# Eclectic-Sheep/sheeprl

Hardware: NVIDIA H100
Metric: Dreamer-V3 train-steps/sec (S, bs16 seq64 horizon15, 64x64x3 obs) (higher is better)
Workload: dtype f32

## Files before the change

sheeprl_b200/csrc/rssm_scan.cu:

```cuda
#include "b200rl.h"
#include "common.cuh"

namespace {

constexpr int SCAN_G = 128;
constexpr int SCAN_NT = 512;
constexpr int SCAN_NW = SCAN_NT / 32;
constexpr int MAXB = 16;
constexpr int MAXRPU = 8;
constexpr int KS_MAX = 8;
constexpr int CLS_SLICES = 8;

typedef unsigned long long u64;

__host__ __device__ inline int r4(int x) { return (x + 3) / 4 * 4; }
__host__ __device__ inline int imax(int a, int b) { return a > b ? a : b; }
__host__ __device__ inline int imin(int a, int b) { return a < b ? a : b; }

__host__ __device__ inline int owned_groups(int width, int cta) {
  const int groups = (width + 3) / 4;
  return (groups > cta) ? (groups - cta + SCAN_G - 1) / SCAN_G : 0;
}
__host__ __device__ inline int owned_cols(int width, int cta) {
  int n = 0;
// ... 147 lines not shown
                make_float2(__uint_as_float((unsigned)a[u]), __uint_as_float((unsigned)b[u]));
      }
    }
  if (!has_s) return;
  while (poll_sums() && !sp.fail()) {}
  float v0 = 0.f, v1 = 0.f;
#pragma unroll
  for (int i = 0; i < SCAN_G / 32; ++i) {
    v0 += __uint_as_float((unsigned)sx[i]);
    v1 += __uint_as_float((unsigned)sy[i]);
  }
  v0 = warp_sum(v0); v1 = warp_sum(v1);
  if (lane == 0) { out1[sr0 + wid] = v0 * inv; out2[sr0 + wid] = v1 * inv; }
}

struct Slot {
  int b, cj, col;
  bool ok;
};
__device__ __forceinline__ Slot make_slot(int e, int per_row, int B, int cta, int width) {
  Slot s;
  s.b = per_row > 0 ? e / per_row : 0;
  s.cj = e - s.b * per_row;
  s.col = (cta + (s.cj >> 2) * SCAN_G) * 4 + (s.cj & 3);
  s.ok = per_row > 0 && s.b < B && s.col < width;
  return s;
}

__device__ __forceinline__ float fsilu(float x) { return __fdividef(x, 1.f + __expf(-x)); }

__device__ __forceinline__ void mma_tf32(float (&d)[4], const unsigned (&a)[4], unsigned b0, unsigned b1) {
  asm volatile("mma.sync.aligned.m16n8k8.row.col.f32.tf32.tf32.f32 {%0,%1,%2,%3}, {%4,%5,%6,%7}, {%8,%9}, {%0,%1,%2,%3};"
               : "+f"(d[0]), "+f"(d[1]), "+f"(d[2]), "+f"(d[3])
               : "r"(a[0]), "r"(a[1]), "r"(a[2]), "r"(a[3]), "r"(b0), "r"(b1));
}
__device__ __forceinline__ unsigned tf32_hi(float x) { return __float_as_uint(x) & 0xffffe000u; }
__device__ __forceinline__ unsigned tf32_lo(float x) { return __float_as_uint(x - __uint_as_float(__float_as_uint(x) & 0xffffe000u)); }

__device__ __forceinline__ void mma_item(const float* __restrict__ X, int xs, int B, const float* __restrict__ w, int wst,
                                         int nvalid, int k0, int k1, float* part, int ldp, int c0, int lane) {
  const int g = lane >> 2, t = lane & 3;
  const bool r_lo = g < B, r_hi = g + 8 < B, n_ok = g < nvalid;
  const float* xa = X + (size_t)g * xs;
  const float* xb = X + (size_t)(g + 8) * xs;
  const float* wr = w + (size_t)g * wst;
  float d[4] = {0.f, 0.f, 0.f, 0.f}, dx[4] = {0.f, 0.f, 0.f, 0.f}, dy[4] = {0.f, 0.f, 0.f, 0.f};
  for (int kb = k0; kb < k1; kb += 16) {
    const int k = kb + 4 * t;
    const bool k_ok = k < k1;
    float4 va = make_float4(0.f, 0.f, 0.f, 0.f), vb = va, vw = va;
    if (r_lo && k_ok) va = *reinterpret_cast<const float4*>(xa + k);
    if (r_hi && k_ok) vb = *reinterpret_cast<const float4*>(xb + k);
    if (n_ok && k_ok) vw = *reinterpret_cast<const float4*>(wr + k);
    {
      const unsigned ah[4] = {tf32_hi(va.x), tf32_hi(vb.x), tf32_hi(va.y), tf32_hi(vb.y)};
      const unsigned al[4] = {tf32_lo(va.x), tf32_lo(vb.x), tf32_lo(va.y), tf32_lo(vb.y)};
      const unsigned bh0 = tf32_hi(vw.x), bh1 = tf32_hi(vw.y), bl0 = tf32_lo(vw.x), bl1 = tf32_lo(vw.y);
      mma_tf32(dx, ah, bl0, bl1);
      mma_tf32(dy, al, bh0, bh1);
      mma_tf32(d, ah, bh0, bh1);
    }
    {
      const unsigned ah[4] = {tf32_hi(va.z), tf32_hi(vb.z), tf32_hi(va.w), tf32_hi(vb.w)};
      const unsigned al[4] = {tf32_lo(va.z), tf32_lo(vb.z), tf32_lo(va.w), tf32_lo(vb.w)};
      const unsigned bh0 = tf32_hi(vw.z), bh1 = tf32_hi(vw.w), bl0 = tf32_lo(vw.z), bl1 = tf32_lo(vw.w);
      mma_tf32(dx, ah, bl0, bl1);
      mma_tf32(dy, al, bh0, bh1);
      mma_tf32(d, ah, bh0, bh1);
    }
  }
#pragma unroll
  for (int i = 0; i < 4; ++i) d[i] += dx[i] + dy[i];
  const int c = 2 * t;
  if (c < nvalid) {
    part[(size_t)g * ldp + c0 + c] = d[0];
    part[(size_t)(g + 8) * ldp + c0 + c] = d[2];
  }
  if (c + 1 < nvalid) {
    part[(size_t)g * ldp + c0 + c + 1] = d[1];
    part[(size_t)(g + 8) * ldp + c0 + c + 1] = d[3];
  }
}

__device__ __forceinline__ int product(const float* X, int xs, const float* wbase, int wst, int ngroups, int K, int B,
                                       float* PART, int ldp, int cbase, int tid) {
  if (ngroups <= 0) return 0;
  const int lane = tid & 31, wid = tid >> 5;
  const int ncols = ngroups * 4, ntiles = (ncols + 7) >> 3, Kp = r4(K);
  int ks = imin(KS_MAX, imax(1, SCAN_NW / ntiles));
  const int kchunk = ((Kp + ks - 1) / ks + 15) / 16 * 16;
  ks = (Kp + kchunk - 1) / kchunk;
  for (int item = wid; item < ntiles * ks; item += SCAN_NW) {
    const int sl = item / ntiles, tile = item - sl * ntiles;
    const int k0 = sl * kchunk, k1 = imin(Kp, k0 + kchunk);
    mma_item(X, xs, B, wbase + (size_t)tile * 8 * wst, wst, imin(8, ncols - tile * 8), k0, k1,
             PART + (size_t)sl * MAXB * ldp, ldp, cbase + tile * 8, lane);
  }
  return ks;
}

__device__ __forceinline__ float part_sum(const float* PART, int ldp, int ks, int b, int c) {
  float v = 0.f;
  for (int s = 0; s < ks; ++s) v += PART[((size_t)s * MAXB + b) * ldp + c];
  return v;
}

__device__ __forceinline__ void class_product(const float* X, int xs, const float* W, int wst, int D, int Kp, int nr, float* PART,
                                              int tid) {
  const int lane = tid & 31, wid = tid >> 5, g = lane >> 2, t = lane & 3;
  const int sl = wid % CLS_SLICES, half = wid / CLS_SLICES;
  const int kc = ((Kp + CLS_SLICES - 1) / CLS_SLICES + 15) / 16 * 16;
  const int k0 = sl * kc, k1 = imin(Kp, k0 + kc);
  const int n0 = half * 16;
  if (n0 >= D) return;
  const bool r_ok = g < nr, n_ok0 = n0 + g < D, n_ok1 = n0 + 8 + g < D;
  const float* xa = X + (size_t)g * xs;
  const float* w0 = W + (size_t)(n0 + g) * wst;
  const float* w1 = W + (size_t)(n0 + 8 + g) * wst;
  float d0[4] = {0.f, 0.f, 0.f, 0.f}, d1[4] = {0.f, 0.f, 0.f, 0.f};
  float e0[4] = {0.f, 0.f, 0.f, 0.f}, e1[4] = {0.f, 0.f, 0.f, 0.f};
  for (int kb = k0; kb < k1; kb += 16) {
    const int k = kb + 4 * t;
    const bool k_ok = k < k1;
    float4 va = make_float4(0.f, 0.f, 0.f, 0.f), v0 = va, v1 = va;
    if (r_ok && k_ok) va = *reinterpret_cast<const float4*>(xa + k);
    if (n_ok0 && k_ok) v0 = *reinterpret_cast<const float4*>(w0 + k);
    if (n_ok1 && k_ok) v1 = *reinterpret_cast<const float4*>(w1 + k);
    {
      const unsigned ah[4] = {tf32_hi(va.x), 0u, tf32_hi(va.y), 0u}, al[4] = {tf32_lo(va.x), 0u, tf32_lo(va.y), 0u};
      mma_tf32(e0, ah, tf32_lo(v0.x), tf32_lo(v0.y)); mma_tf32(e1, ah, tf32_lo(v1.x), tf32_lo(v1.y));
      mma_tf32(d0, ah, tf32_hi(v0.x), tf32_hi(v0.y)); mma_tf32(d1, ah, tf32_hi(v1.x), tf32_hi(v1.y));
      mma_tf32(e0, al, tf32_hi(v0.x), tf32_hi(v0.y)); mma_tf32(e1, al, tf32_hi(v1.x), tf32_hi(v1.y));
    }
    {
      const unsigned ah[4] = {tf32_hi(va.z), 0u, tf32_hi(va.w), 0u}, al[4] = {tf32_lo(va.z), 0u, tf32_lo(va.w), 0u};
      mma_tf32(e0, ah, tf32_lo(v0.z), tf32_lo(v0.w)); mma_tf32(e1, ah, tf32_lo(v1.z), tf32_lo(v1.w));
      mma_tf32(d0, ah, tf32_hi(v0.z), tf32_hi(v0.w)); mma_tf32(d1, ah, tf32_hi(v1.z), tf32_hi(v1.w));
      mma_tf32(e0, al, tf32_hi(v0.z), tf32_hi(v0.w)); mma_tf32(e1, al, tf32_hi(v1.z), tf32_hi(v1.w));
    }
  }
  if (g < nr) {
    float* out = PART + ((size_t)sl * MAXRPU + g) * 32 + n0 + 2 * t;
    out[0] = d0[0] + e0[0]; out[1] = d0[1] + e0[1];
    out[8] = d1[0] + e1[0]; out[9] = d1[1] + e1[1];
  }
}

__device__ __forceinline__ void load_rows4(float* dst, int wst, int koff, const float* W, size_t ld, int row0, int nrows_valid,
                                           int c0, int K, int Kp, int tid) {
  for (int j = 0; j < 4; ++j)
    for (int k = tid; k < Kp; k += SCAN_NT)
      dst[j * wst + koff + k] = (row0 + j < nrows_valid && k < K) ? W[(size_t)(row0 + j) * ld + c0 + k] : 0.f;
}
__device__ __forceinline__ void load_cols4(float* dst, int wst, const float* W, size_t ld, int col0, int ncols_valid,
                                           int K, int koff, int tid) {
  for (int e = tid; e < K * 4; e += SCAN_NT) {
    const int k = e >> 2, j = e & 3;
    dst[j * wst + koff + k] = (col0 + j < ncols_valid) ? W[(size_t)k * ld + col0 + j] : 0.f;
  }
}

__device__ __forceinline__ void prof_mark(long long* prof, int slot, long long& last, bool on) {
  if (on) {
    const long long now = clock64();
    prof[slot] += now - last;
    last = now;
  }
}

struct GeoF {
  int ngh, ngr, ngx;
  int sR, sDx, sDr, wgst, w2st;
  int nsplit, rpu;
  int unit_g, unit_r0, unit_nr;
  int ldp;
  int kin;
  int oWg, oWr1, oW2, oWin, oXh, oXx, oPart, oAcc, oX0, oPar, oMisc, oInt, total;
};

struct Dims { int B, S, D, R, Dx, Dr, A; };

// ... 333 lines not shown
      prof_mark(prof, 10, tlast, prof_on);
      {
        const int nrp = nr <= 1 ? 1 : (nr <= 2 ? 2 : (nr <= 4 ? 4 : 8));
        const int wpr = SCAN_NW / nrp, bb = wid / wpr, wi = wid - bb * wpr;
        float* xr = Xx + bb * xxs;
        float s = 0.f, q2 = 0.f;
        if (bb < nr)
          for (int k = wi * 32 + lane; k < Dr; k += wpr * 32) { const float xv = xr[k]; s += xv; q2 = fmaf(xv, xv, q2); }
        s = warp_sum(s);
        q2 = warp_sum(q2);
        if (lane == 0) { misc[48 + wid] = s; misc[80 + wid] = q2; }
        __syncthreads();
        float mu = 0.f, var = 0.f;
        for (int i = 0; i < wpr; ++i) { mu += misc[48 + bb * wpr + i]; var += misc[80 + bb * wpr + i]; }
        mu /= (float)Dr;
        var = fmaxf(var / (float)Dr - mu * mu, 0.f);
        const float rstd = rsqrtf(var + a.eps);
        if (bb < nr) {
          for (int k = wi * 32 + lane; k < Dr; k += wpr * 32) {
            const float o = fsilu((xr[k] - mu) * rstd * LNRG[k] + LNRB[k]);
            xr[k] = o;
            if (gq == 0) a.rp_act[(row0 + rb + bb) * Dr + k] = o;
          }
          if (gq == 0 && wi == 0 && lane == 0) {
            ws.ln_stats[((size_t)2 * NB + row0 + rb + bb) * 2] = mu;
            ws.ln_stats[((size_t)2 * NB + row0 + rb + bb) * 2 + 1] = rstd;
          }
        }
      }
      __syncthreads();
      prof_mark(prof, 14, tlast, prof_on);
      class_product(Xx, xxs, W2, g.w2st, D, g.sDr, nr, PART, tid);
      __syncthreads();
      prof_mark(prof, 15, tlast, prof_on);
      if (wid < nr) {
        const int bb = wid, b = rb + bb;
        const bool on = lane < D;
        float lg = 0.f;
        for (int s2 = 0; s2 < CLS_SLICES; ++s2) lg += PART[((size_t)s2 * MAXRPU + bb) * 32 + lane];
        const float raw = on ? lg + bias2 : -INFINITY;
        const float mx = warp_max(raw);
        const float ex = on ? expf(raw - mx) : 0.f;
        const float se = warp_sum(ex);
        float pmc = ex / se, l = raw;
        if (a.unimix > 0.f) {
          pmc = fminf(fmaxf((1.f - a.unimix) * pmc + a.unimix / (float)D, kFp32Eps), 1.f - kFp32Eps);
          l = logf(pmc);
        }
        float best = on ? pmc / noise_pref : -INFINITY;
        int besti = on ? lane : 0x7fffffff;
#pragma unroll
        for (int s2 = 16; s2 > 0; s2 >>= 1) {
          const float ob = __shfl_xor_sync(0xffffffffu, best, s2);
          const int oi = __shfl_xor_sync(0xffffffffu, besti, s2);
          if (ob > best || (ob == best && oi < besti)) { best = ob; besti = oi; }
        }
        if (lane == 0) ll_store(ws.ll + L.z + ((size_t)par * MAXB + b) * S + gq, __uint_as_float((unsigned)besti), tag);
        const size_t o = (row0 + b) * Z + (size_t)gq * D + lane;
        if (lane == 0) ws.zidx[(row0 + b) * S + gq] = besti;
        if (on) {
          a.post_raw[o] = raw;
          a.post_mix[o] = l;
          const float zt = (lane == besti) ? 1.f : 0.f;
          a.latent[(row0 + b) * a.ld_lat + (size_t)gq * D + lane] = zt;
          if (t + 1 < T)
            a.z_in[(row0 + B + b) * Z + (size_t)gq * D + lane] = (1.f - fnext) * zt + fnext * ((z0idx[gq] == lane) ? 1.f : 0.f);
        }
      }
      prof_mark(prof, 11, tlast, prof_on);
    }
    __syncthreads();
    if (sp.dead) break;
  }
  if (prof_on)
    for (int i = 0; i < 32; ++i) ws.prof[cta * 32 + i] = sprof[i];
}

struct GeoB {
  int ngh, ngx, ngr;
  int sZ, sR, sDx, sDr, xw;
  int wgst, winst;
  int nsplit, rpu, unit_g, unit_r0, unit_nr;
  int ldp;
  int oW2, oW1, oWg, oWin, oX, oPart, oAcc, oSt, oDhc, oDh0, oWs, oMisc, total;
};

__host__ __device__ inline GeoB make_geo_b(const Dims& a, int cta) {
  GeoB g;
  const int Z = a.S * a.D;
  g.ngh = owned_groups(a.R, cta);
  g.ngx = owned_groups(a.Dx, cta);
  g.ngr = owned_groups(a.Dr, cta);
  g.sZ = r4(Z); g.sR = r4(a.R); g.sDx = r4(a.Dx); g.sDr = r4(a.Dr);
  g.xw = imax(imax(g.sZ, 2 * g.sR), imax(g.sDx, g.sDr));
  g.wgst = 3 * g.sR;
  g.winst = g.sDx + 4;
  g.nsplit = imax(1, imin(a.B, SCAN_G / a.S));
  g.rpu = (a.B + g.nsplit - 1) / g.nsplit;
  g.unit_g = -1; g.unit_r0 = 0; g.unit_nr = 0;
  if (cta < a.S * g.nsplit) {
    const int sp = cta / a.S;
    g.unit_r0 = sp * g.rpu;
    g.unit_nr = imin(g.rpu, a.B - g.unit_r0);
    if (g.unit_nr > 0) g.unit_g = cta % a.S; else g.unit_nr = 0;
  }
  const int mh = owned_groups(a.R, 0), mx = owned_groups(a.Dx, 0), mr = owned_groups(a.Dr, 0);
  g.ldp = imax(imax((mh + mx) * 4, mr * 4), 4);
  int o = 0;
  g.oW2 = o;   o += mr * 4 * g.sZ;
  g.oW1 = o;   o += mh * 4 * g.sDr;
  g.oWg = o;   o += (mh + mx) * 4 * g.wgst;
  g.oWin = o;  o += a.D * g.winst;
  g.oX = o;    o += MAXB * g.xw;
  g.oPart = o; o += imax(KS_MAX * MAXB * g.ldp, CLS_SLICES * MAXRPU * 32);
  g.oAcc = o;  o += MAXB * g.ldp;
  g.oSt = o;   o += 2 * MAXB * imax(imax(mh * 12, mx * 4), imax(mr * 4, 4));
  g.oDhc = o;  o += MAXB * imax(mh * 4, 4);
  g.oDh0 = o;  o += imax(mh * 4, 4);
  g.oWs = o;   o += mh * 4 + (mh + mx) * 4 + 32;
  g.oMisc = o; o += 16 * MAXB + 64;
  g.total = o;
  return g;
}

__device__ __forceinline__ void send_row_sums(const float* ST, int ncols, int B, u64* base, int par, int cta, unsigned tag, int tid) {
  const int lane = tid & 31, wid = tid >> 5;
  for (int b = wid; b < B; b += SCAN_NW) {
    float s1 = 0.f, s2 = 0.f;
    for (int c = lane; c < ncols; c += 32) { s1 += ST[(b * ncols + c) * 2]; s2 += ST[(b * ncols + c) * 2 + 1]; }
    s1 = warp_sum(s1); s2 = warp_sum(s2);
    if (lane == 0) ll_store2(base + (((size_t)par * MAXB + b) * SCAN_G + cta) * 2, s1, s2, tag);
  }
}

template <bool FIX>
__global__ void __launch_bounds__(SCAN_NT, 1)
rssm_scan_bwd_kernel(const b200rl_rssm_scan_args a, const b200rl_rssm_scan_grads q) {
  extern __shared__ __align__(16) float sm[];
  const int tid = threadIdx.x, lane = tid & 31, wid = tid >> 5;
  const int cta = blockIdx.x;
  const int T = a.T, B = a.B;
  const int S = FIX ? 32 : a.S, D = FIX ? 32 : a.D, Z = S * D, R = FIX ? 512 : a.R, Dx = FIX ? 512 : a.Dx, Dr = FIX ? 512 : a.Dr;
  const int KG = R + Dx, KIN = Z + a.A, NB = T * B;
  const GeoB g = make_geo_b(Dims{B, S, D, R, Dx, Dr, a.A}, cta);
  const Workspace ws = carve(a.workspace, T, B, S, D, Dx, R, Dr);
  const LLGeo L = make_ll(S, Dx, R, Dr, Z);
  const int mh = owned_groups(R, 0), mx = owned_groups(Dx, 0);
  float* W2T = sm + g.oW2;
  float* W1T = sm + g.oW1;
  float* WgT = sm + g.oWg;
  float* WinU = sm + g.oWin;
  float* X = sm + g.oX;
  float* PART = sm + g.oPart;
  float* ACC = sm + g.oAcc;
  float* ST = sm + g.oSt;
  float* DHC = sm + g.oDhc;
  float* DH0 = sm + g.oDh0;
  float* WS1 = sm + g.oWs;
  float* WSG = WS1 + mh * 4;
  float* WSI = WSG + (mh + mx) * 4;
  float* misc = sm + g.oMisc;
  float* S1 = misc + 32;
  float* S2 = misc + 48;
  float* LNS = misc + 64;
  float* LNX1 = misc + 64 + 6 * MAXB;
  const int xw = g.xw, ldp = g.ldp;
  const int nh4 = g.ngh * 4, nx4 = g.ngx * 4, nr4 = g.ngr * 4;
  const bool unit = g.unit_g >= 0;
  __shared__ long long sprof[32];
  const bool prof_on = (cta < 2) && tid == 0;
  long long* prof = sprof;
  if (tid < 32) sprof[tid] = 0;
  long long tlast = prof_on ? clock64() : 0;
  Spin sp;
  sp.init(ws.error);

  for (int e = tid; e < g.total; e += SCAN_NT) sm[e] = 0.f;
  __syncthreads();
  for (int gi = 0; gi < g.ngr; ++gi)
    load_cols4(W2T + (size_t)gi * 4 * g.sZ, g.sZ, a.W_r2, Dr, (cta + gi * SCAN_G) * 4, Dr, Z, 0, tid);
  for (int gi = 0; gi < g.ngh; ++gi) {
    const int c0 = (cta + gi * SCAN_G) * 4;
    load_cols4(W1T + (size_t)gi * 4 * g.sDr, g.sDr, a.W_r1, a.ld_wr1, c0, R, Dr, 0, tid);
    for (int part = 0; part < 3; ++part)
      load_cols4(WgT + (size_t)gi * 4 * g.wgst, g.wgst, a.W_g + (size_t)part * R * KG, KG, c0, R, R, part * g.sR, tid);
  }
  for (int gi = 0; gi < g.ngx; ++gi)
    for (int part = 0; part < 3; ++part)
      load_cols4(WgT + (size_t)(g.ngh + gi) * 4 * g.wgst, g.wgst, a.W_g + (size_t)part * R * KG + R, KG,
                 (cta + gi * SCAN_G) * 4, Dx, R, part * g.sR, tid);
  if (unit)
    for (int e = tid; e < D * Dx; e += SCAN_NT) {
      const int c = e / D, d = e - c * D;
      WinU[d * g.winst + c] = a.W_in[(size_t)c * KIN + g.unit_g * D + d];
    }
  __syncthreads();
  for (int j = wid; j < nh4; j += SCAN_NW) {
    float s = 0.f;
    for (int k = lane; k < g.sDr; k += 32) s += W1T[(size_t)j * g.sDr + k];
    s = warp_sum(s);
    if (lane == 0) WS1[j] = s;
  }
  for (int j = wid; j < nh4 + nx4; j += SCAN_NW) {
    float s = 0.f;
    for (int k = lane; k < g.wgst; k += 32) s += WgT[(size_t)j * g.wgst + k];
    s = warp_sum(s);
    if (lane == 0) WSG[j] = s;
  }
  if (unit)
    for (int d = wid; d < D; d += SCAN_NW) {
      float s = 0.f;
      for (int k = lane; k < g.sDx; k += 32) s += WinU[(size_t)d * g.winst + k];
      s = warp_sum(s);
      if (lane == 0) WSI[d] = s;
    }
  __syncthreads();
  const Slot sR_ = make_slot(tid, nr4, B, cta, Dr);
  const Slot sH = make_slot(tid, nh4, B, cta, R);
  const Slot sX = make_slot(tid, nx4, B, cta, Dx);
  const float gam_r = sR_.ok ? a.lnr_g[sR_.col] : 0.f, bet_r = sR_.ok ? a.lnr_b[sR_.col] : 0.f;
  const float gam_x = sX.ok ? a.lnx_g[sX.col] : 0.f, bet_x = sX.ok ? a.lnx_b[sX.col] : 0.f;
  float gam_g[3] = {0.f, 0.f, 0.f};
  if (sH.ok)
#pragma unroll
    for (int part = 0; part < 3; ++part) gam_g[part] = a.lng_g[part * R + sH.col];
  const float ws1 = sH.ok ? WS1[sH.cj] : 0.f, wsgh = sH.ok ? WSG[sH.cj] : 0.f, wsgx = sX.ok ? WSG[nh4 + sX.cj] : 0.f;
  const float wsi = (unit && lane < D) ? WSI[lane] : 0.f;
  float dh0_acc = 0.f;
  prof_mark(prof, 16, tlast, prof_on);

  for (int t = T - 1; t >= 0; --t) {
    const size_t row0 = (size_t)t * B;
    const int bt = T - 1 - t, par = bt & 1;
    const unsigned tag = (unsigned)bt + 1u;
    const bool last = (t == T - 1);

    if (tid < MAXB) {
      misc[tid] = (tid < B) ? a.first[row0 + tid] : 0.f;
      misc[16 + tid] = (tid < B && !last) ? a.first[row0 + B + tid] : 0.f;
    }
    for (int e = tid; e < 3 * B * 2; e += SCAN_NT) {
      const int which = e / (B * 2), r_ = e - which * (B * 2);
      LNS[which * MAXB * 2 + r_] = ws.ln_stats[((size_t)which * NB + row0) * 2 + r_];
    }
    if (!last)
      for (int e = tid; e < B * 2; e += SCAN_NT) LNX1[e] = ws.ln_stats[((size_t)0 * NB + row0 + B) * 2 + e];
    const float p_rp = sR_.ok ? a.rp_pre[(row0 + sR_.b) * Dr + sR_.col] : 0.f;
    float p_hin = 0.f, p_dlh = 0.f, p_qr = 0.f, p_qgh = 0.f, p_gl[3] = {0.f, 0.f, 0.f}, p_gp[3] = {0.f, 0.f, 0.f};
    if (sH.ok) {
      p_hin = a.h_in[(row0 + sH.b) * R + sH.col];
      p_dlh = q.d_latent[(row0 + sH.b) * a.ld_lat + Z + sH.col];
      p_qr = q.q_r[(row0 + sH.b) * R + sH.col];
      p_qgh = q.q_g[(row0 + sH.b) * KG + sH.col];
#pragma unroll
      for (int part = 0; part < 3; ++part) {
        p_gl[part] = a.g_ln[(row0 + sH.b) * 3 * R + part * R + sH.col];
        p_gp[part] = a.g_pre[(row0 + sH.b) * 3 * R + part * R + sH.col];
      }
    }
    const float p_xp = sX.ok ? a.x_pre[(row0 + sX.b) * Dx + sX.col] : 0.f;
    const float p_qgx = sX.ok ? q.q_g[(row0 + sX.b) * KG + R + sX.col] : 0.f;
    float u_dl = 0.f, u_dmix = 0.f, u_raw = -INFINITY, u_qx = 0.f;
    if (unit && wid < g.unit_nr && lane < D) {
      const size_t o = (row0 + g.unit_r0 + wid) * Z + (size_t)g.unit_g * D + lane;
      u_dl = q.d_latent[(row0 + g.unit_r0 + wid) * a.ld_lat + (size_t)g.unit_g * D + lane];
      u_dmix = q.d_post_mix[o];
      u_raw = a.post_raw[o];
      if (!last) u_qx = q.q_x[(row0 + B + g.unit_r0 + wid) * Z + (size_t)g.unit_g * D + lane];
    }
    __syncthreads();
    const float* fl = misc;

    if (unit) {
      const int gq = g.unit_g, nr = g.unit_nr, rb = g.unit_r0;
      if (!last) {
        ll_recv<4>(X, xw, ws.ll + L.d + ((size_t)(par ^ 1) * MAXB + rb) * Dx, Dx, nr, Dx, (unsigned)bt, tid, sp,
                   ws.ll + L.sd + (size_t)(par ^ 1) * MAXB * SCAN_G * 2, rb, 1.f / (float)Dx, S1, S2);
        __syncthreads();
        prof_mark(prof, 17, tlast, prof_on);
        class_product(X, xw, WinU, g.winst, D, g.sDx, nr, PART, tid);
        __syncthreads();
      }
      if (wid < nr) {
        const int bb = wid, b = rb + bb;
        const bool on = lane < D;
        float dz = u_dl;
        if (!last) {
          float p1 = 0.f;
          for (int s2 = 0; s2 < CLS_SLICES; ++s2) p1 += PART[((size_t)s2 * MAXRPU + bb) * 32 + lane];
          if (on) {
            const float mu = LNX1[b * 2], rstd = LNX1[b * 2 + 1];
            const float p2 = rstd * (u_qx - mu * wsi);
            dz += (1.f - fl[16 + b]) * rstd * (p1 - S1[b] * wsi - S2[b] * p2);
          }
        }
        const float mx_ = warp_max(u_raw);
        const float ex = on ? expf(u_raw - mx_) : 0.f;
        const float sft = ex / warp_sum(ex);
        float gg = u_dmix;
        if (a.unimix > 0.f) {
          const float pmx = (1.f - a.unimix) * sft + a.unimix / (float)D;
          const float pmc = on ? fminf(fmaxf(pmx, kFp32Eps), 1.f - kFp32Eps) : 0.f;
          const float p = pmc / warp_sum(pmc);
          const float pdz = warp_sum(p * dz);
          gg += p * (dz - pdz);
          const bool inside = on && pmx >= kFp32Eps && pmx <= 1.f - kFp32Eps;
          const float ds = inside ? gg * (1.f - a.unimix) / pmx : 0.f;
          const float sds = warp_sum(sft * ds);
          gg = sft * (ds - sds);
        } else {
          const float pdz = warp_sum(sft * dz);
          gg += sft * (dz - pdz);
        }
        if (on) {
          ll_store(ws.ll + L.a + ((size_t)par * MAXB + b) * Z + (size_t)gq * D + lane, gg, tag);
          q.d_post_raw[(row0 + b) * Z + (size_t)gq * D + lane] = gg;
        }
      }
      prof_mark(prof, 18, tlast, prof_on);
    }

    __syncthreads();
    ll_recv<4>(X, xw, ws.ll + L.a + (size_t)par * MAXB * Z, Z, B, Z, tag, tid, sp);
    __syncthreads();
    prof_mark(prof, 19, tlast, prof_on);
    const int ks2 = product(X, xw, W2T, g.sZ, g.ngr, Z, B, PART, ldp, 0, tid);
    __syncthreads();
    float dact_r = 0.f;
    if (sR_.ok) {
      dact_r = part_sum(PART, ldp, ks2, sR_.b, sR_.cj);
      const float xh = (p_rp - LNS[(2 * MAXB + sR_.b) * 2]) * LNS[(2 * MAXB + sR_.b) * 2 + 1];
      const float ln = xh * gam_r + bet_r;
      const float sg = sigmoidf_(ln);
      const float dxh = dact_r * sg * (1.f + ln * (1.f - sg)) * gam_r;
      ll_store(ws.ll + L.b + ((size_t)par * MAXB + sR_.b) * Dr + sR_.col, dxh, tag);
      ST[(sR_.b * nr4 + sR_.cj) * 2] = dxh;
      ST[(sR_.b * nr4 + sR_.cj) * 2 + 1] = dxh * xh;
    } else if (tid < B * nr4) {
      ST[tid * 2] = 0.f; ST[tid * 2 + 1] = 0.f;
    }
    __syncthreads();
    send_row_sums(ST, nr4, B, ws.ll + L.sb, par, cta, tag, tid);
    if (sR_.ok) q.d_rp_act[(row0 + sR_.b) * Dr + sR_.col] = dact_r;
    prof_mark(prof, 20, tlast, prof_on);

    __syncthreads();
    ll_recv<4>(X, xw, ws.ll + L.b + (size_t)par * MAXB * Dr, Dr, B, Dr, tag, tid, sp,
               ws.ll + L.sb + (size_t)par * MAXB * SCAN_G * 2, 0, 1.f / (float)Dr, S1, S2);
    __syncthreads();
    prof_mark(prof, 21, tlast, prof_on);
    const int ks1 = product(X, xw, W1T, g.sDr, g.ngh, Dr, B, PART, ldp, 0, tid);
    __syncthreads();
    float dhin_gate = 0.f, dgl[3] = {0.f, 0.f, 0.f};
    if (sH.ok) {
      const int b = sH.b;
      const float mur = LNS[(2 * MAXB + b) * 2], rstdr = LNS[(2 * MAXB + b) * 2 + 1];
      const float mug = LNS[(1 * MAXB + b) * 2], rstdg = LNS[(1 * MAXB + b) * 2 + 1];
      const float p1 = part_sum(PART, ldp, ks1, b, sH.cj);
      const float p2 = rstdr * (p_qr - mur * ws1);
      float dh = p_dlh + rstdr * (p1 - S1[b] * ws1 - S2[b] * p2);
      if (!last) dh += DHC[b * nh4 + sH.cj];
      const float r = sigmoidf_(p_gl[0]), cnd = tanhf(r * p_gl[1]), u = sigmoidf_(p_gl[2] - 1.f);
      const float du = dh * (cnd - p_hin);
      const float drc = dh * u * (1.f - cnd * cnd);
      dgl[0] = drc * p_gl[1] * r * (1.f - r);
      dgl[1] = drc * r;
      dgl[2] = du * u * (1.f - u);
      dhin_gate = dh * (1.f - u);
#pragma unroll
      for (int part = 0; part < 3; ++part) {
        const float xh = (p_gp[part] - mug) * rstdg;
        const float dxh = dgl[part] * gam_g[part];
        ll_store(ws.ll + L.c + ((size_t)par * MAXB + b) * 3 * R + (size_t)part * R + sH.col, dxh, tag);
        ST[(b * (3 * nh4) + part * nh4 + sH.cj) * 2] = dxh;
        ST[(b * (3 * nh4) + part * nh4 + sH.cj) * 2 + 1] = dxh * xh;
      }
    } else if (tid < B * nh4) {
      const int b = tid / imax(nh4, 1), cj = tid - b * nh4;
#pragma unroll
      for (int part = 0; part < 3; ++part) {
        ST[(b * (3 * nh4) + part * nh4 + cj) * 2] = 0.f;
        ST[(b * (3 * nh4) + part * nh4 + cj) * 2 + 1] = 0.f;
      }
    }
    __syncthreads();
    send_row_sums(ST, 3 * nh4, B, ws.ll + L.sc, par, cta, tag, tid);
    if (sH.ok)
#pragma unroll
      for (int part = 0; part < 3; ++part) q.d_g_ln[(row0 + sH.b) * 3 * R + part * R + sH.col] = dgl[part];
    prof_mark(prof, 22, tlast, prof_on);

    __syncthreads();
    for (int part = 0; part < 2; ++part)
      ll_recv<4>(X + part * g.sR, xw, ws.ll + L.c + (size_t)par * MAXB * 3 * R + (size_t)part * R, 3 * R, B, R, tag, tid, sp);
    __syncthreads();
    const int ksa = product(X, xw, WgT, g.wgst, g.ngh + g.ngx, 2 * g.sR, B, PART, ldp, 0, tid);
    __syncthreads();
    float acc_h = sH.ok ? part_sum(PART, ldp, ksa, sH.b, sH.cj) : 0.f;
    float acc_x = sX.ok ? part_sum(PART, ldp, ksa, sX.b, nh4 + sX.cj) : 0.f;
    __syncthreads();
    ll_recv<4>(X, xw, ws.ll + L.c + (size_t)par * MAXB * 3 * R + (size_t)2 * R, 3 * R, B, R, tag, tid, sp,
               ws.ll + L.sc + (size_t)par * MAXB * SCAN_G * 2, 0, 1.f / (float)(3 * R), S1, S2);
    __syncthreads();
    const int ksb = product(X, xw, WgT + 2 * g.sR, g.wgst, g.ngh + g.ngx, R, B, PART, ldp, 0, tid);
    __syncthreads();
    prof_mark(prof, 23, tlast, prof_on);
    float dact_x = 0.f;
    if (sX.ok) {
      const int b = sX.b;
      acc_x += part_sum(PART, ldp, ksb, b, nh4 + sX.cj);
      const float mug = LNS[(1 * MAXB + b) * 2], rstdg = LNS[(1 * MAXB + b) * 2 + 1];
      const float mux = LNS[(0 * MAXB + b) * 2], rstdx = LNS[(0 * MAXB + b) * 2 + 1];
      const float p2 = rstdg * (p_qgx - mug * wsgx);
      dact_x = rstdg * (acc_x - S1[b] * wsgx - S2[b] * p2);
      const float xh = (p_xp - mux) * rstdx;
      const float ln = xh * gam_x + bet_x;
      const float sg = sigmoidf_(ln);
      const float dxh = dact_x * sg * (1.f + ln * (1.f - sg)) * gam_x;
      ll_store(ws.ll + L.d + ((size_t)par * MAXB + b) * Dx + sX.col, dxh, tag);
      ST[(b * nx4 + sX.cj) * 2] = dxh;
      ST[(b * nx4 + sX.cj) * 2 + 1] = dxh * xh;
    } else if (tid < B * nx4) {
      ST[tid * 2] = 0.f; ST[tid * 2 + 1] = 0.f;
    }
    float dhin_f = 0.f;
    if (sH.ok) {
      const int b = sH.b;
      acc_h += part_sum(PART, ldp, ksb, b, sH.cj);
      const float mug = LNS[(1 * MAXB + b) * 2], rstdg = LNS[(1 * MAXB + b) * 2 + 1];
      const float p2 = rstdg * (p_qgh - mug * wsgh);
      const float dhin = dhin_gate + rstdg * (acc_h - S1[b] * wsgh - S2[b] * p2);
      DHC[b * nh4 + sH.cj] = (1.f - fl[b]) * dhin;
      dhin_f = fl[b] * dhin;
    }
    __syncthreads();
    send_row_sums(ST, nx4, B, ws.ll + L.sd, par, cta, tag, tid);
    if (sX.ok) q.d_x_act[(row0 + sX.b) * Dx + sX.col] = dact_x;
    if (sH.ok) ACC[sH.b * ldp + sH.cj] = dhin_f;
    __syncthreads();
    if (tid < nh4)
      for (int b = 0; b < B; ++b)
        if (fl[b] != 0.f) dh0_acc += ACC[b * ldp + tid];
    prof_mark(prof, 24, tlast, prof_on);
    __syncthreads();
    if (sp.dead) break;
  }
  if (tid < nh4) {
    const int col = (cta + (tid >> 2) * SCAN_G) * 4 + (tid & 3);
    if (col < R) q.d_h0[col] = dh0_acc;
  }
  (void)DH0;
  if (prof_on)
    for (int i = 0; i < 32; ++i) ws.prof[cta * 32 + i] = sprof[i];
}

bool fixed_dims(const b200rl_rssm_scan_args& a) { return a.S == 32 && a.D == 32 && a.R == 512 && a.Dx == 512 && a.Dr == 512; }

size_t scan_smem(const b200rl_rssm_scan_args& a, bool backward) {
  const Dims d{a.B, a.S, a.D, a.R, a.Dx, a.Dr, a.A};
  return sizeof(float) * (size_t)(backward ? make_geo_b(d, 0).total : make_geo_f(d, 0).total);
}

int scan_check(const b200rl_rssm_scan_args& a, bool backward) {
  RL_CHECK_ARG(a.B >= 1 && a.B <= MAXB, "persistent scan supports batch <= 16 rows per rank");
  RL_CHECK_ARG(a.D >= 1 && a.D <= 32, "persistent scan supports <= 32 classes per categorical");
  RL_CHECK_ARG(a.T >= 1 && a.S >= 1 && a.S <= 64, "persistent scan supports T >= 1 and 1 <= S <= 64 categoricals");
  RL_CHECK_ARG(a.Dx % 2 == 0 && a.R % 2 == 0 && a.Dr % 2 == 0 && (a.S * a.D) % 2 == 0, "persistent scan supports even layer widths");
  RL_CHECK_ARG(a.Dx <= 1024, "persistent scan supports recurrent dense_units <= 1024");
  RL_CHECK_ARG(MAXB * owned_groups(a.R, 0) * 12 <= SCAN_NT, "persistent scan supports recurrent_state_size <= 1024");
  RL_CHECK_ARG(MAXB * owned_groups(a.Dr, 0) * 4 <= SCAN_NT, "persistent scan supports representation hidden_size <= 4096");
  RL_CHECK_ARG(scan_smem(a, backward) <= 227 * 1024, "weight slices do not fit in shared memory for this model size");
  return B200RL_OK;
}

int workspace_check(const b200rl_rssm_scan_args& a) {
  RL_CHECK_ARG(a.workspace && a.workspace_bytes >= (long long)ws_bytes(a.T, a.B, a.S, a.D, a.Dx, a.R, a.Dr), "workspace too small");
  return B200RL_OK;
}

struct GruLL { size_t s, h, c, sc, total; };
__host__ __device__ inline GruLL make_gru_ll(int R) {
  GruLL g;
  size_t o = 0;
  g.s = o;  o += 2 * (size_t)MAXB * SCAN_G * 2;
  g.h = o;  o += 2 * (size_t)MAXB * R;
  g.c = o;  o += 2 * (size_t)MAXB * 3 * R;
  g.sc = o; o += 2 * (size_t)MAXB * SCAN_G * 2;
  g.total = o;
  return g;
}
__host__ __device__ inline size_t gru_ws_bytes(int T, int B, int R) {
  return WS_HEADER + make_gru_ll(R).total * sizeof(u64) + sizeof(float) * 2 * (size_t)T * B + 256;
}

struct GeoG {
  int ngh, sR, ldp;
  int pw;
  int oW, oX, oPart, oAcc, oSt, oDhc, oPar, oLn, oMisc, oTab, total;
};
__host__ __device__ inline GeoG make_geo_g(int R, int cta, bool backward) {
  GeoG g;
  g.ngh = owned_groups(R, cta);
  g.sR = r4(R);
  const int mh = owned_groups(R, 0);
  g.ldp = backward ? mh * 4 : mh * 12;
  for (g.pw = backward ? 3 : 1;; g.pw = 1) {
    int o = 0;
    g.oW = o;    o += mh * 12 * g.sR;
    g.oX = o;    o += MAXB * g.pw * g.sR;
    g.oPart = o; o += KS_MAX * MAXB * g.ldp;
    g.oAcc = o;  o += MAXB * g.ldp;
    g.oSt = o;   o += backward ? 2 * MAXB * mh * 12 : 0;
// ... 393 lines not shown
```

Before: 62.17.

## Fuse gate-gradient products and poll low-latency flags inside the MMA loop

The backward scan's two sequential gate-gradient products (first two gate parts, then the third part after a separate receive) become one fused work list. Warps consume the third part directly from the tagged low-latency buffer, polling the tags inside the MMA item, which removes a receive phase and two block barriers per timestep. LayerNorm gamma/beta and weight sums move from registers into shared memory to relieve register pressure. The PART buffer doubles in size, which raises shared memory use, and spin-polling inside warps could serialize on slow producers.

```diff
diff --git a/sheeprl_b200/csrc/rssm_scan.cu b/sheeprl_b200/csrc/rssm_scan.cu
--- a/sheeprl_b200/csrc/rssm_scan.cu
+++ b/sheeprl_b200/csrc/rssm_scan.cu
@@ -253,14 +253,104 @@
   }
 }
 
+template <int LL_STEPS>
+__device__ __forceinline__ void mma_item_ll(const u64* src, int ss, int kvalid, int B, const float* __restrict__ w, int wst,
+                                            int nvalid, int k0, int k1, float* part, int ldp, int c0, int lane, unsigned tag,
+                                            Spin& sp) {
+  const int g = lane >> 2, t = lane & 3;
+  const bool r_lo = g < B, r_hi = g + 8 < B, n_ok = g < nvalid;
+  const u64* xa = src + (size_t)g * ss;
+  const u64* xb = src + (size_t)(g + 8) * ss;
+  const float* wr = w + (size_t)g * wst;
+  float d[4] = {0.f, 0.f, 0.f, 0.f}, dx[4] = {0.f, 0.f, 0.f, 0.f}, dy[4] = {0.f, 0.f, 0.f, 0.f};
+  const u64 zero = ll_pack(0.f, tag);
+  for (int kb0 = k0; kb0 < k1; kb0 += 16 * LL_STEPS) {
+    u64 e[LL_STEPS][8];
+    auto polled = [&](int s, int p) {
+      const int k = kb0 + 16 * s + 4 * t + 2 * (p & 1);
+      return ((p >> 1) ? r_hi : r_lo) && k < k1 && k < kvalid;
+    };
+    auto load = [&](int s, int p) {
+      const int k = kb0 + 16 * s + 4 * t + 2 * (p & 1);
+      ll_load2(((p >> 1) ? xb : xa) + k, e[s][2 * p], e[s][2 * p + 1]);
+    };
+#pragma unroll
+    for (int s = 0; s < LL_STEPS; ++s)
+#pragma unroll
+      for (int p = 0; p < 4; ++p) {
+        if (polled(s, p)) load(s, p);
+        else e[s][2 * p] = e[s][2 * p + 1] = zero;
+      }
+    for (;;) {
+      bool stale = false;
+#pragma unroll
+      for (int s = 0; s < LL_STEPS; ++s)
+#pragma unroll
+        for (int i = 0; i < 8; ++i) stale |= (unsigned)(e[s][i] >> 32) != tag;
+      if (!stale || sp.fail()) break;
+#pragma unroll
+      for (int s = 0; s < LL_STEPS; ++s)
+#pragma unroll
+        for (int p = 0; p < 4; ++p)
+          if ((unsigned)(e[s][2 * p] >> 32) != tag || (unsigned)(e[s][2 * p + 1] >> 32) != tag) load(s, p);
+    }
+    __syncwarp();
+#pragma unroll
+    for (int s = 0; s < LL_STEPS; ++s) {
+      const int kb = kb0 + 16 * s;
+      if (kb >= k1) break;
+      const int k = kb + 4 * t;
+      float4 vw = make_float4(0.f, 0.f, 0.f, 0.f);
+      if (n_ok && k < k1) vw = *reinterpret_cast<const float4*>(wr + k);
+      const float4 va = make_float4(__uint_as_float((unsigned)e[s][0]), __uint_as_float((unsigned)e[s][1]),
+                                    __uint_as_float((unsigned)e[s][2]), __uint_as_float((unsigned)e[s][3]));
+      const float4 vb = make_float4(__uint_as_float((unsigned)e[s][4]), __uint_as_float((unsigned)e[s][5]),
+                                    __uint_as_float((unsigned)e[s][6]), __uint_as_float((unsigned)e[s][7]));
+      {
+        const unsigned ah[4] = {tf32_hi(va.x), tf32_hi(vb.x), tf32_hi(va.y), tf32_hi(vb.y)};
+        const unsigned al[4] = {tf32_lo(va.x), tf32_lo(vb.x), tf32_lo(va.y), tf32_lo(vb.y)};
+        const unsigned bh0 = tf32_hi(vw.x), bh1 = tf32_hi(vw.y), bl0 = tf32_lo(vw.x), bl1 = tf32_lo(vw.y);
+        mma_tf32(dx, ah, bl0, bl1);
+        mma_tf32(dy, al, bh0, bh1);
+        mma_tf32(d, ah, bh0, bh1);
+      }
+      {
+        const unsigned ah[4] = {tf32_hi(va.z), tf32_hi(vb.z), tf32_hi(va.w), tf32_hi(vb.w)};
+        const unsigned al[4] = {tf32_lo(va.z), tf32_lo(vb.z), tf32_lo(va.w), tf32_lo(vb.w)};
+        const unsigned bh0 = tf32_hi(vw.z), bh1 = tf32_hi(vw.w), bl0 = tf32_lo(vw.z), bl1 = tf32_lo(vw.w);
+        mma_tf32(dx, ah, bl0, bl1);
+        mma_tf32(dy, al, bh0, bh1);
+        mma_tf32(d, ah, bh0, bh1);
+      }
+    }
+  }
+#pragma unroll
+  for (int i = 0; i < 4; ++i) d[i] += dx[i] + dy[i];
+  const int c = 2 * t;
+  if (c < nvalid) {
+    part[(size_t)g * ldp + c0 + c] = d[0];
+    part[(size_t)(g + 8) * ldp + c0 + c] = d[2];
+  }
+  if (c + 1 < nvalid) {
+    part[(size_t)g * ldp + c0 + c + 1] = d[1];
+    part[(size_t)(g + 8) * ldp + c0 + c + 1] = d[3];
+  }
+}
+
+__device__ __forceinline__ void slicing(int ntiles, int K, int& ks, int& kchunk) {
+  const int Kp = r4(K);
+  ks = imin(KS_MAX, imax(1, SCAN_NW / ntiles));
+  kchunk = ((Kp + ks - 1) / ks + 15) / 16 * 16;
+  ks = (Kp + kchunk - 1) / kchunk;
+}
+
 __device__ __forceinline__ int product(const float* X, int xs, const float* wbase, int wst, int ngroups, int K, int B,
                                        float* PART, int ldp, int cbase, int tid) {
   if (ngroups <= 0) return 0;
   const int lane = tid & 31, wid = tid >> 5;
   const int ncols = ngroups * 4, ntiles = (ncols + 7) >> 3, Kp = r4(K);
-  int ks = imin(KS_MAX, imax(1, SCAN_NW / ntiles));
-  const int kchunk = ((Kp + ks - 1) / ks + 15) / 16 * 16;
-  ks = (Kp + kchunk - 1) / kchunk;
+  int ks, kchunk;
+  slicing(ntiles, K, ks, kchunk);
   for (int item = wid; item < ntiles * ks; item += SCAN_NW) {
     const int sl = item / ntiles, tile = item - sl * ntiles;
     const int k0 = sl * kchunk, k1 = imin(Kp, k0 + kchunk);
@@ -268,6 +358,35 @@
              PART + (size_t)sl * MAXB * ldp, ldp, cbase + tile * 8, lane);
   }
   return ks;
+}
+
+template <int LL_STEPS>
+__device__ __forceinline__ void product2(const float* X, int xs, int K1, const u64* src, int ss, int K2, int wofs2, unsigned tag,
+                                         Spin& sp, const float* wbase, int wst, int ngroups, int B, float* PART, int ldp, int tid,
+                                         int& ks1, int& ks2) {
+  ks1 = ks2 = 0;
+  if (ngroups <= 0) return;
+  const int lane = tid & 31, wid = tid >> 5;
+  const int ncols = ngroups * 4, ntiles = (ncols + 7) >> 3;
+  int kc1, kc2;
+  slicing(ntiles, K1, ks1, kc1);
+  slicing(ntiles, K2, ks2, kc2);
+  const int n1 = ntiles * ks1;
+  for (int item = wid; item < n1 + ntiles * ks2; item += SCAN_NW) {
+    const bool second = item >= n1;
+    const int it = second ? item - n1 : item;
+    const int sl = it / ntiles, tile = it - sl * ntiles;
+    const float* w = wbase + (size_t)tile * 8 * wst;
+    const int nvalid = imin(8, ncols - tile * 8);
+    if (second) {
+      const int k0 = sl * kc2, k1 = imin(r4(K2), k0 + kc2);
+      mma_item_ll<LL_STEPS>(src, ss, K2, B, w + wofs2, wst, nvalid, k0, k1, PART + (size_t)(ks1 + sl) * MAXB * ldp, ldp, tile * 8,
+                  lane, tag, sp);
+    } else {
+      const int k0 = sl * kc1, k1 = imin(r4(K1), k0 + kc1);
+      mma_item(X, xs, B, w, wst, nvalid, k0, k1, PART + (size_t)sl * MAXB * ldp, ldp, tile * 8, lane);
+    }
+  }
 }
 
 __device__ __forceinline__ float part_sum(const float* PART, int ldp, int ks, int b, int c) {
@@ -767,7 +886,7 @@
   int wgst, winst;
   int nsplit, rpu, unit_g, unit_r0, unit_nr;
   int ldp;
-  int oW2, oW1, oWg, oWin, oX, oPart, oAcc, oSt, oDhc, oDh0, oWs, oMisc, total;
+  int oW2, oW1, oWg, oWin, oX, oPart, oAcc, oSt, oDhc, oDh0, oWs, oLnp, oMisc, total;
 };
 
 __host__ __device__ inline GeoB make_geo_b(const Dims& a, int cta) {
@@ -797,12 +916,13 @@
   g.oWg = o;   o += (mh + mx) * 4 * g.wgst;
   g.oWin = o;  o += a.D * g.winst;
   g.oX = o;    o += MAXB * g.xw;
-  g.oPart = o; o += imax(KS_MAX * MAXB * g.ldp, CLS_SLICES * MAXRPU * 32);
+  g.oPart = o; o += imax(2 * KS_MAX * MAXB * g.ldp, CLS_SLICES * MAXRPU * 32);
   g.oAcc = o;  o += MAXB * g.ldp;
-  g.oSt = o;   o += 2 * MAXB * imax(imax(mh * 12, mx * 4), imax(mr * 4, 4));
+  g.oSt = o;  o += 2 * MAXB * imax(imax(mh * 12, mx * 4), imax(mr * 4, 4));
   g.oDhc = o;  o += MAXB * imax(mh * 4, 4);
   g.oDh0 = o;  o += imax(mh * 4, 4);
   g.oWs = o;   o += mh * 4 + (mh + mx) * 4 + 32;
+  g.oLnp = o;  o += 2 * mr * 4 + 2 * mx * 4 + 3 * mh * 4;
   g.oMisc = o; o += 16 * MAXB + 64;
   g.total = o;
   return g;
@@ -844,6 +964,9 @@
   float* WS1 = sm + g.oWs;
   float* WSG = WS1 + mh * 4;
   float* WSI = WSG + (mh + mx) * 4;
+  float* GAMR = sm + g.oLnp;
+  float* GAMX = GAMR + 2 * owned_groups(Dr, 0) * 4;
+  float* GAMG = GAMX + 2 * mx * 4;
   float* misc = sm + g.oMisc;
   float* S1 = misc + 32;
   float* S2 = misc + 48;
@@ -903,14 +1026,12 @@
   const Slot sR_ = make_slot(tid, nr4, B, cta, Dr);
   const Slot sH = make_slot(tid, nh4, B, cta, R);
   const Slot sX = make_slot(tid, nx4, B, cta, Dx);
-  const float gam_r = sR_.ok ? a.lnr_g[sR_.col] : 0.f, bet_r = sR_.ok ? a.lnr_b[sR_.col] : 0.f;
-  const float gam_x = sX.ok ? a.lnx_g[sX.col] : 0.f, bet_x = sX.ok ? a.lnx_b[sX.col] : 0.f;
-  float gam_g[3] = {0.f, 0.f, 0.f};
-  if (sH.ok)
-#pragma unroll
-    for (int part = 0; part < 3; ++part) gam_g[part] = a.lng_g[part * R + sH.col];
-  const float ws1 = sH.ok ? WS1[sH.cj] : 0.f, wsgh = sH.ok ? WSG[sH.cj] : 0.f, wsgx = sX.ok ? WSG[nh4 + sX.cj] : 0.f;
-  const float wsi = (unit && lane < D) ? WSI[lane] : 0.f;
+  const int mr4 = owned_groups(Dr, 0) * 4;
+  if (sR_.ok && sR_.b == 0) { GAMR[sR_.cj] = a.lnr_g[sR_.col]; GAMR[mr4 + sR_.cj] = a.lnr_b[sR_.col]; }
+  if (sX.ok && sX.b == 0) { GAMX[sX.cj] = a.lnx_g[sX.col]; GAMX[mx * 4 + sX.cj] = a.lnx_b[sX.col]; }
+  if (sH.ok && sH.b == 0)
+#pragma unroll
+    for (int part = 0; part < 3; ++part) GAMG[part * mh * 4 + sH.cj] = a.lng_g[part * R + sH.col];
   float dh0_acc = 0.f;
   prof_mark(prof, 16, tlast, prof_on);
 
@@ -975,6 +1096,7 @@
           for (int s2 = 0; s2 < CLS_SLICES; ++s2) p1 += PART[((size_t)s2 * MAXRPU + bb) * 32 + lane];
           if (on) {
             const float mu = LNX1[b * 2], rstd = LNX1[b * 2 + 1];
+            const float wsi = WSI[lane];
             const float p2 = rstd * (u_qx - mu * wsi);
             dz += (1.f - fl[16 + b]) * rstd * (p1 - S1[b] * wsi - S2[b] * p2);
           }
@@ -1015,7 +1137,7 @@
     if (sR_.ok) {
       dact_r = part_sum(PART, ldp, ks2, sR_.b, sR_.cj);
       const float xh = (p_rp - LNS[(2 * MAXB + sR_.b) * 2]) * LNS[(2 * MAXB + sR_.b) * 2 + 1];
-      const float ln = xh * gam_r + bet_r;
+      const float gam_r = GAMR[sR_.cj], ln = xh * gam_r + GAMR[mr4 + sR_.cj];
       const float sg = sigmoidf_(ln);
       const float dxh = dact_r * sg * (1.f + ln * (1.f - sg)) * gam_r;
       ll_store(ws.ll + L.b + ((size_t)par * MAXB + sR_.b) * Dr + sR_.col, dxh, tag);
@@ -1042,6 +1164,7 @@
       const float mur = LNS[(2 * MAXB + b) * 2], rstdr = LNS[(2 * MAXB + b) * 2 + 1];
       const float mug = LNS[(1 * MAXB + b) * 2], rstdg = LNS[(1 * MAXB + b) * 2 + 1];
       const float p1 = part_sum(PART, ldp, ks1, b, sH.cj);
+      const float ws1 = WS1[sH.cj];
       const float p2 = rstdr * (p_qr - mur * ws1);
       float dh = p_dlh + rstdr * (p1 - S1[b] * ws1 - S2[b] * p2);
       if (!last) dh += DHC[b * nh4 + sH.cj];
@@ -1055,7 +1178,7 @@
 #pragma unroll
       for (int part = 0; part < 3; ++part) {
         const float xh = (p_gp[part] - mug) * rstdg;
-        const float dxh = dgl[part] * gam_g[part];
+        const float dxh = dgl[part] * GAMG[part * mh * 4 + sH.cj];
         ll_store(ws.ll + L.c + ((size_t)par * MAXB + b) * 3 * R + (size_t)part * R + sH.col, dxh, tag);
         ST[(b * (3 * nh4) + part * nh4 + sH.cj) * 2] = dxh;
         ST[(b * (3 * nh4) + part * nh4 + sH.cj) * 2 + 1] = dxh * xh;
@@ -1076,30 +1199,30 @@
     prof_mark(prof, 22, tlast, prof_on);
 
     __syncthreads();
-    for (int part = 0; part < 2; ++part)
-      ll_recv<4>(X + part * g.sR, xw, ws.ll + L.c + (size_t)par * MAXB * 3 * R + (size_t)part * R, 3 * R, B, R, tag, tid, sp);
-    __syncthreads();
-    const int ksa = product(X, xw, WgT, g.wgst, g.ngh + g.ngx, 2 * g.sR, B, PART, ldp, 0, tid);
-    __syncthreads();
+    const u64* dxh_g = ws.ll + L.c + (size_t)par * MAXB * 3 * R;
+    ll_recv<4>(X, xw, dxh_g, 3 * R, B, R, tag, tid, sp);
+    ll_recv<4>(X + g.sR, xw, dxh_g + R, 3 * R, B, R, tag, tid, sp, ws.ll + L.sc + (size_t)par * MAXB * SCAN_G * 2, 0,
+               1.f / (float)(3 * R), S1, S2);
+    __syncthreads();
+    prof_mark(prof, 25, tlast, prof_on);
+    int ksa, ksb;
+    product2<FIX ? 2 : 1>(X, xw, 2 * g.sR, dxh_g + 2 * R, 3 * R, R, 2 * g.sR, tag, sp, WgT, g.wgst, g.ngh + g.ngx, B, PART, ldp, tid, ksa, ksb);
+    __syncthreads();
+    prof_mark(prof, 23, tlast, prof_on);
+    const float* PARTB = PART + (size_t)ksa * MAXB * ldp;
     float acc_h = sH.ok ? part_sum(PART, ldp, ksa, sH.b, sH.cj) : 0.f;
     float acc_x = sX.ok ? part_sum(PART, ldp, ksa, sX.b, nh4 + sX.cj) : 0.f;
-    __syncthreads();
-    ll_recv<4>(X, xw, ws.ll + L.c + (size_t)par * MAXB * 3 * R + (size_t)2 * R, 3 * R, B, R, tag, tid, sp,
-               ws.ll + L.sc + (size_t)par * MAXB * SCAN_G * 2, 0, 1.f / (float)(3 * R), S1, S2);
-    __syncthreads();
-    const int ksb = product(X, xw, WgT + 2 * g.sR, g.wgst, g.ngh + g.ngx, R, B, PART, ldp, 0, tid);
-    __syncthreads();
-    prof_mark(prof, 23, tlast, prof_on);
     float dact_x = 0.f;
     if (sX.ok) {
       const int b = sX.b;
-      acc_x += part_sum(PART, ldp, ksb, b, nh4 + sX.cj);
+      acc_x += part_sum(PARTB, ldp, ksb, b, nh4 + sX.cj);
       const float mug = LNS[(1 * MAXB + b) * 2], rstdg = LNS[(1 * MAXB + b) * 2 + 1];
       const float mux = LNS[(0 * MAXB + b) * 2], rstdx = LNS[(0 * MAXB + b) * 2 + 1];
+      const float wsgx = WSG[nh4 + sX.cj];
       const float p2 = rstdg * (p_qgx - mug * wsgx);
       dact_x = rstdg * (acc_x - S1[b] * wsgx - S2[b] * p2);
       const float xh = (p_xp - mux) * rstdx;
-      const float ln = xh * gam_x + bet_x;
+      const float gam_x = GAMX[sX.cj], ln = xh * gam_x + GAMX[mx * 4 + sX.cj];
       const float sg = sigmoidf_(ln);
       const float dxh = dact_x * sg * (1.f + ln * (1.f - sg)) * gam_x;
       ll_store(ws.ll + L.d + ((size_t)par * MAXB + b) * Dx + sX.col, dxh, tag);
@@ -1111,8 +1234,9 @@
     float dhin_f = 0.f;
     if (sH.ok) {
       const int b = sH.b;
-      acc_h += part_sum(PART, ldp, ksb, b, sH.cj);
+      acc_h += part_sum(PARTB, ldp, ksb, b, sH.cj);
       const float mug = LNS[(1 * MAXB + b) * 2], rstdg = LNS[(1 * MAXB + b) * 2 + 1];
+      const float wsgh = WSG[sH.cj];
       const float p2 = rstdg * (p_qgh - mug * wsgh);
       const float dhin = dhin_gate + rstdg * (acc_h - S1[b] * wsgh - S2[b] * p2);
       DHC[b * nh4 + sH.cj] = (1.f - fl[b]) * dhin;
```

Result: no change. 62.39, median of 6 (+0.4%).
